# MechaCritter/Python-Visual-Similarity

Hardware: AMD Instinct MI355X
Metric: images/sec encoded + top-k retrieved, VLAD K256 RootSIFT (higher is better)
Workload: dtype f32

## Files before the change

include/pvsim.h:

```cpp
#ifndef PVSIM_H
#define PVSIM_H

#include <stddef.h>
#include <stdint.h>

#ifdef __cplusplus
extern "C" {
#endif

#define PVS_VERSION 103

typedef enum {
  PVS_OK = 0,
  PVS_ERR_INVALID = 1,
  PVS_ERR_NO_DEVICE = 2,
  PVS_ERR_OOM = 3,
  PVS_ERR_UNSUPPORTED = 4,
  PVS_ERR_DIM = 5
} pvs_status;

typedef enum {
  PVS_DESC_F32 = 0,
  PVS_DESC_F32_ROOTSIFT = 1,
  PVS_DESC_U8_ROOTSIFT = 2
} pvs_desc_kind;

typedef enum {
  PVS_OPT_ASSIGN_PREFILTER = 0,
  PVS_OPT_VLAD_PATH = 1,
  PVS_OPT_TOPK_SELECT_ONLY = 2,
  PVS_OPT_AGG_VARIANT = 3,
  PVS_OPT_FISHER_SCALE = 4,
  PVS_OPT_COUNT_ = 5
} pvs_option;

typedef struct pvs_ctx pvs_ctx;
typedef struct pvs_codebook pvs_codebook;
typedef struct pvs_gmm pvs_gmm;
typedef struct pvs_pca pvs_pca;
typedef struct pvs_comm pvs_comm;

typedef struct {
  double power_norm_weight;
  double norm_order;
  double epsilon;
} pvs_norm_params;

int pvs_version(void);
const char* pvs_last_error(void);
int pvs_device_count(int* count);
int pvs_init(int device_id, void* stream, pvs_ctx** out);
int pvs_destroy(pvs_ctx* ctx);
int pvs_sync(pvs_ctx* ctx);
void* pvs_stream(pvs_ctx* ctx);
int pvs_device_name(pvs_ctx* ctx, char* buf, size_t buflen);
int pvs_set_option(pvs_ctx* ctx, int option, int value);
int pvs_get_option(pvs_ctx* ctx, int option, int* value);

int pvs_malloc(pvs_ctx* ctx, size_t bytes, void** dptr);
int pvs_free(pvs_ctx* ctx, void* dptr);
int pvs_memcpy_h2d(pvs_ctx* ctx, void* dst_dev, const void* src_host, size_t bytes);
int pvs_memcpy_d2h(pvs_ctx* ctx, void* dst_host, const void* src_dev, size_t bytes);
int pvs_memset(pvs_ctx* ctx, void* dst_dev, int value, size_t bytes);

int pvs_fill_dev(pvs_ctx* ctx, void* dst_dev, int64_t n_elems, int elem_bytes, uint64_t pattern);
int pvs_stream_wait(pvs_ctx* waiter, pvs_ctx* signal);

int pvs_codebook_create(pvs_ctx* ctx, const float* centroids , int K, int D, pvs_codebook** out);
int pvs_codebook_destroy(pvs_ctx* ctx, pvs_codebook* cb);
int pvs_gmm_create(pvs_ctx* ctx, const double* weights , const double* means ,
                   const double* covariances , int K, int D, pvs_gmm** out);
int pvs_gmm_destroy(pvs_ctx* ctx, pvs_gmm* g);
int pvs_pca_create(pvs_ctx* ctx, const float* components , const float* mean ,
                   int n_components, int d_in, pvs_pca** out);
int pvs_pca_destroy(pvs_ctx* ctx, pvs_pca* p);

int pvs_vlad_encode(pvs_ctx* ctx, const pvs_codebook* cb, const pvs_pca* pca, const void* desc,
                    int desc_kind, const int64_t* offsets, int64_t n_images, const pvs_norm_params* prm,
                    float* out, int32_t* out_labels);
int pvs_vlad_encode_dev(pvs_ctx* ctx, const pvs_codebook* cb, const pvs_pca* pca, const void* d_desc,
                        int desc_kind, const int64_t* d_offsets, int64_t n_images, int64_t total_desc,
                        const pvs_norm_params* prm, float* d_out, int32_t* d_labels, float* d_inv_norm);
int pvs_kmeans_predict_dev(pvs_ctx* ctx, const pvs_codebook* cb, const void* d_desc, int desc_kind,
                           int64_t total_desc, int32_t* d_labels);

int pvs_fisher_encode(pvs_ctx* ctx, const pvs_gmm* g, const pvs_pca* pca, const void* desc, int desc_kind,
                      const int64_t* offsets, int64_t n_images, const pvs_norm_params* prm, double* out);
int pvs_fisher_encode_dev(pvs_ctx* ctx, const pvs_gmm* g, const pvs_pca* pca, const void* d_desc,
                          int desc_kind, const int64_t* d_offsets, int64_t n_images, int64_t total_desc,
                          const pvs_norm_params* prm, void* d_out, int out_f64);
int pvs_gmm_predict_proba_dev(pvs_ctx* ctx, const pvs_gmm* g, const void* d_desc, int desc_kind,
                              int64_t total_desc, double* d_resp);
int pvs_pca_transform_dev(pvs_ctx* ctx, const pvs_pca* p, const void* d_desc, int desc_kind,
                          int64_t total_desc, float* d_out);

int pvs_cosine(pvs_ctx* ctx, const void* A, int64_t M, const void* B, int64_t N, int64_t L, int is_f64,
               void* out );
int pvs_row_inv_norms_dev(pvs_ctx* ctx, const float* d_x, int64_t rows, int64_t L, float* d_inv);
int pvs_cosine_dev(pvs_ctx* ctx, const float* d_A, int64_t M, const float* d_B, int64_t N, int64_t L,
                   const float* d_inv_a, const float* d_inv_b, float* d_out, int64_t ldo);

int pvs_cosine_dual_dev(pvs_ctx* ctx, const float* d_A, int64_t M, const float* d_B, int64_t N, int64_t L,
                        const float* d_inv_a, const float* d_inv_b, float* d_out, int64_t ldo, float* d_out_t, int64_t ldt);

int pvs_topk_dev(pvs_ctx* ctx, const float* d_scores, int64_t nq, int64_t ncols, int64_t ld, int k,
                 int64_t col_offset, int merge, int64_t* d_idx, float* d_val);
int pvs_cosine_topk_dev(pvs_ctx* ctx, const float* d_Q, int64_t nq, const float* d_DB, int64_t N, int64_t L,
                        const float* d_inv_q, const float* d_inv_db, int k, int64_t col_offset, int merge,
                        int64_t* d_idx, float* d_val);
int pvs_f32_to_f16_dev(pvs_ctx* ctx, const float* d_src, int64_t n, void* d_dst_f16);
int pvs_cosine_f16_dev(pvs_ctx* ctx, const void* d_A16, int64_t M, const void* d_B16, int64_t N, int64_t L,
                       const float* d_inv_a, const float* d_inv_b, float* d_out, int64_t ldo);
int pvs_cosine_topk_f16_dev(pvs_ctx* ctx, const void* d_Q16, int64_t nq, const void* d_DB16, int64_t N, int64_t L,
                            const float* d_inv_q, const float* d_inv_db, int k, int64_t col_offset, int merge,
                            int64_t* d_idx, float* d_val);
int pvs_cosine_topk(pvs_ctx* ctx, const float* Q, int64_t nq, const float* DB, int64_t N, int64_t L, int k,
// ... 62 lines not shown
```

python-visual-similarity_amd/csrc/common.hpp:

```cpp
#pragma once
#include <hip/hip_runtime.h>

#include <cmath>
#include <cstdarg>
#include <cstdint>
#include <cstdio>
#include <cstring>
#include <map>
#include <vector>

#include "../../include/pvsim.h"
#include "../../include/pvsim_diag.h"

#define PVS_EXPORT extern "C" __attribute__((visibility("default")))

namespace pvs {

void set_error(const char* fmt, ...);

#define PVS_FAIL(code, ...)        \
  do {                             \
    ::pvs::set_error(__VA_ARGS__); \
    return (code);                 \
  } while (0)

#define PVS_HIP(expr)                                                                    \
  do {                                                                                   \
    hipError_t e__ = (expr);                                                             \
    if (e__ != hipSuccess) {                                                             \
      ::pvs::set_error("%s failed: %s (%s:%d)", #expr, hipGetErrorString(e__), __FILE__, \
                       __LINE__);                                                        \
      return e__ == hipErrorOutOfMemory ? PVS_ERR_OOM : PVS_ERR_NO_DEVICE;               \
    }                                                                                    \
  } while (0)

#define PVS_TRY(expr)                 \
  do {                                \
    int s__ = (expr);                 \
    if (s__ != PVS_OK) return s__;    \
  } while (0)

constexpr int WAVE = 64;

enum TimerSlot { T_ASSIGN = 0, T_AGGREGATE = 1, T_GEMM = 2, T_TOPK = 3, T_FPOST = 4, T_FMOM = 5, T_MISC = 6, T_RESCORE = 7 };

struct TimerRec {
  hipEvent_t a, b;
  int slot;
};

}

struct pvs_ctx {
  int device = 0;
  hipStream_t stream = nullptr;
  bool owns_stream = false;
  int num_cu = 256;
  static constexpr int NWS = 9;
  void* ws[NWS] = {};
  size_t ws_bytes[NWS] = {};
  struct GemmPlanSlot {
    int key[4] = {-1, -1, -1, -1};
    int n_main = 0, n_tail = 0, splitk = 1;
    void* d_tiles = nullptr;
    size_t cap = 0;
  } gemm_plan[5];
  std::map<const void*, int> lds_attr;
  int opt[PVS_OPT_COUNT_] = {1, 0, 0, 0, 0};
  unsigned int* d_queue = nullptr;
  unsigned long long* d_fused_stamps = nullptr;
  bool timers_on = false;
  std::vector<pvs::TimerRec> pending;
  std::vector<hipEvent_t> event_pool;
  std::multimap<size_t, void*> block_cache;
  std::map<void*, size_t> block_size;
  size_t block_cache_bytes = 0;
  void* h_stage = nullptr;
  size_t h_stage_bytes = 0;
  double t_total[PVS_TIMER_SLOTS] = {0};
  int64_t t_count[PVS_TIMER_SLOTS] = {0};
};

struct pvs_codebook {
  int K = 0, D = 0;
  int K_pad = 0, D_pad = 0;
  float* d_cent = nullptr;
  float* d_cpad = nullptr;
  float* d_cnorm = nullptr;
  void* d_c16 = nullptr;
  int D_pad16 = 0;
  int c16_shift = 0;
  float cmax = 0.f;
  void* d_cnk = nullptr;
  void* d_c16n = nullptr;
  int cn_e1 = 0;
};

struct pvs_gmm {
  int K = 0, D = 0;
  double* d_w = nullptr;
  double* d_mu = nullptr;
  double* d_cov = nullptr;
  double* d_prec = nullptr;
  double* d_mup = nullptr;
  double* d_inv_mu = nullptr;
  double* d_inv_sg = nullptr;
  double* d_const = nullptr;
};

struct pvs_pca {
  int C = 0, Din = 0;
  float* d_comp = nullptr;
  float* d_off = nullptr;
};

namespace pvs {

int ws_reserve(pvs_ctx* ctx, int which, size_t bytes, void** out);

inline int ensure_lds(pvs_ctx* ctx, const void* fn, size_t bytes) {
  auto it = ctx->lds_attr.find(fn);
  if (it == ctx->lds_attr.end() || it->second < (int)bytes) {
    PVS_HIP(hipFuncSetAttribute(fn, hipFuncAttributeMaxDynamicSharedMemorySize, (int)bytes));
    ctx->lds_attr[fn] = (int)bytes;
  }
  return PVS_OK;
}

struct ScopedTimer {
  pvs_ctx* ctx;
  int slot;
  hipEvent_t a = nullptr, b = nullptr;
  hipEvent_t take_event() {
    if (!ctx->event_pool.empty()) {
      hipEvent_t e = ctx->event_pool.back();
      ctx->event_pool.pop_back();
      return e;
    }
    hipEvent_t e = nullptr;
    return hipEventCreate(&e) == hipSuccess ? e : nullptr;
  }
  ScopedTimer(pvs_ctx* c, int s) : ctx(c), slot(s) {
    if (ctx->timers_on) {
      if (ctx->pending.size() >= 128) {
        size_t done = 0;
        while (done < ctx->pending.size() && hipEventQuery(ctx->pending[done].b) == hipSuccess) {
          float ms = 0.f;
          if (hipEventElapsedTime(&ms, ctx->pending[done].a, ctx->pending[done].b) == hipSuccess) {
            ctx->t_total[ctx->pending[done].slot] += ms;
            ctx->t_count[ctx->pending[done].slot] += 1;
          }
// ... 78 lines not shown
```

python-visual-similarity_amd/csrc/vlad.hip:

```cpp
#include "common.hpp"
#include "desc_load.hpp"

namespace pvs {

typedef float f32x16 __attribute__((ext_vector_type(16)));

struct AssignArgs {
  const void* X;
  int64_t total;
  int D, ld;
  const float* Cpad;
  const float* cnorm;
  int K_pad, D_pad;
  int32_t* labels;
  const int64_t* rows;
  const unsigned long long* nrows;
  int64_t rows_cap;
};

constexpr int ASSIGN_THREADS = 512;
constexpr int ASSIGN_ROWS = (ASSIGN_THREADS / 64) * 32;
constexpr int ASSIGN_DCHUNK = 128;

template <int NT, int KIND, bool VEC>
__global__ __launch_bounds__(ASSIGN_THREADS, 2) void assign_kernel(AssignArgs a) {
  extern __shared__ __attribute__((aligned(16))) char smem[];
  constexpr int CB = 32 * NT;
  const int cw_max = a.D_pad < ASSIGN_DCHUNK ? a.D_pad : ASSIGN_DCHUNK;
  const int stride = cw_max + 4;
  float* lds_c = reinterpret_cast<float*>(smem);
  float* lds_n = lds_c + CB * stride;

  const int lane = threadIdx.x & 63, wave = threadIdx.x >> 6;
  const int j = lane & 31, h = lane >> 5;
  const int ncb = a.K_pad / CB;
  const int nsc = (a.D_pad + ASSIGN_DCHUNK - 1) / ASSIGN_DCHUNK;
  const bool restage = (ncb * nsc) > 1;
  const int64_t n_items = a.rows ? (int64_t)a.nrows[blockIdx.x] : a.total;
  const int64_t nblocks = (n_items + ASSIGN_ROWS - 1) / ASSIGN_ROWS;
  const int64_t* const my_rows = a.rows ? a.rows + (int64_t)blockIdx.x * a.rows_cap : nullptr;

  auto stage = [&](int cb, int sc) {
    const int cw = min(ASSIGN_DCHUNK, a.D_pad - sc * ASSIGN_DCHUNK);
    const int c4n = cw >> 2;
    for (int idx = threadIdx.x; idx < CB * c4n; idx += ASSIGN_THREADS) {
      const int r = idx / c4n, c4 = idx - r * c4n;
      const float4 v = *reinterpret_cast<const float4*>(a.Cpad + (int64_t)(cb * CB + r) * a.D_pad +
                                                        sc * ASSIGN_DCHUNK + 4 * c4);
      *reinterpret_cast<float4*>(lds_c + r * stride + 4 * c4) = v;
    }
    for (int idx = threadIdx.x; idx < CB; idx += ASSIGN_THREADS) lds_n[idx] = a.cnorm[cb * CB + idx];
  };

  if (!restage) {
    stage(0, 0);
    __syncthreads();
  }

  for (int64_t blk = my_rows ? 0 : blockIdx.x; blk < nblocks; blk += my_rows ? 1 : gridDim.x) {
    const int64_t item = blk * ASSIGN_ROWS + wave * 32 + j;
    const bool rvalid = item < n_items;
    const int64_t row = (my_rows && rvalid) ? my_rows[item] : item;
    float best = INFINITY;
    int bidx = 0;

    for (int cb = 0; cb < ncb; ++cb) {
      f32x16 acc[NT];
#pragma unroll
      for (int t = 0; t < NT; ++t)
#pragma unroll
        for (int r = 0; r < 16; ++r) acc[t][r] = 0.f;

      for (int sc = 0; sc < nsc; ++sc) {
        if (restage) {
          __syncthreads();
          stage(cb, sc);
          __syncthreads();
        }
        const int dc = sc * ASSIGN_DCHUNK;
        const int nt = min(ASSIGN_DCHUNK, a.D_pad - dc) >> 3;

        float4 xb[16];
#pragma unroll
        for (int t = 0; t < 16; ++t) {
          xb[t] = make_float4(0.f, 0.f, 0.f, 0.f);
          if (t < nt) {
            const int d = dc + 8 * t + 4 * h;
            if constexpr (VEC) {
              if (rvalid && d < a.D) xb[t] = load4<KIND>(a.X, row, a.ld, d);
            } else {
              if (rvalid) {
                if (d + 0 < a.D) xb[t].x = load1<KIND>(a.X, row, a.ld, d + 0);
                if (d + 1 < a.D) xb[t].y = load1<KIND>(a.X, row, a.ld, d + 1);
                if (d + 2 < a.D) xb[t].z = load1<KIND>(a.X, row, a.ld, d + 2);
                if (d + 3 < a.D) xb[t].w = load1<KIND>(a.X, row, a.ld, d + 3);
              }
            }
          }
        }
        if constexpr (DescTraits<KIND>::rootsift) {
          float s = 0.f;
#pragma unroll
          for (int t = 0; t < 16; ++t) s += (xb[t].x + xb[t].y) + (xb[t].z + xb[t].w);
          s += __shfl_xor(s, 32, 64);
          const RootsiftRow<KIND> rr(s);
#pragma unroll
          for (int t = 0; t < 16; ++t) {
            xb[t].x = rr(xb[t].x);
            xb[t].y = rr(xb[t].y);
            xb[t].z = rr(xb[t].z);
            xb[t].w = rr(xb[t].w);
          }
        }

#pragma unroll
        for (int t = 0; t < 16; ++t) {
          if (t < nt) {
#pragma unroll
            for (int tile = 0; tile < NT; ++tile) {
              const float4 c4 =
                  *reinterpret_cast<const float4*>(lds_c + (32 * tile + j) * stride + 8 * t + 4 * h);
// ... 655 lines not shown
            for (int tile = 0; tile < 2; ++tile)
#pragma unroll
              for (int f = 0; f < 2; ++f)
                acc[ab][tile][f] = __builtin_amdgcn_mfma_f32_16x16x32_f16(fl[buf][tile], xh[f][s], s == 0 ? zero4 : acc[ab][tile][f], 0, 0, 0);
          }
          if constexpr (NP >= 2) {
#pragma unroll
            for (int tile = 0; tile < 2; ++tile)
#pragma unroll
              for (int f = 0; f < 2; ++f)
                acc[ab][tile][f] = __builtin_amdgcn_mfma_f32_16x16x32_f16(fh[buf][tile], xl[f][s], (NP == 2 && s == 0) ? zero4 : acc[ab][tile][f], 0, 0, 0);
          }
#pragma unroll
          for (int tile = 0; tile < 2; ++tile)
#pragma unroll
            for (int f = 0; f < 2; ++f)
              acc[ab][tile][f] = __builtin_amdgcn_mfma_f32_16x16x32_f16(fh[buf][tile], xh[f][s], (NP == 1 && s == 0) ? zero4 : acc[ab][tile][f], 0, 0, 0);
          if (s == 3) {
#pragma unroll
            for (int tile = 0; tile < 2; ++tile) {
              const f16x4_t pk = *reinterpret_cast<const f16x4_t*>(lds_k + 4 * (32 * gr + 16 * tile + j));
              f16x8_t ca;
#pragma unroll
              for (int q = 0; q < 8; ++q) ca[q] = (_Float16)0.f;
              if constexpr (LUT) {
                if (g == 0) { ca[0] = pk[0]; ca[1] = pk[0]; ca[2] = pk[1]; ca[3] = pk[1]; ca[4] = pk[2]; ca[5] = pk[2]; }
              } else {
                if (g == 0) { ca[0] = pk[0]; ca[1] = pk[1]; ca[2] = pk[2]; }
              }
#pragma unroll
              for (int f = 0; f < 2; ++f)
                acc[ab][tile][f] = __builtin_amdgcn_mfma_f32_16x16x32_f16(ca, cnb[f], acc[ab][tile][f], 0, 0, 0);
            }
          }
          if (gr > 0) select4(ab ^ 1, gr - 1, s);
          __builtin_amdgcn_sched_barrier(0);
        }
      }
    }
#pragma unroll
    for (int part = 0; part < 4; ++part) select4(1, 7, part);
    __builtin_amdgcn_s_barrier();

#pragma unroll
    for (int f = 0; f < 2; ++f) {
      const float m2s = -2.f * ldexpf(1.f, -(x_shift[f] + a.c_shift));
      float b = best[f] * m2s, sc = second[f] * m2s;
      int bi = bidx[f] + 4 * g;
#pragma unroll
      for (int m = 16; m <= 32; m <<= 1) {
        const float ob = __shfl_xor(b, m, 64), os = __shfl_xor(sc, m, 64);
        const int oi = __shfl_xor(bi, m, 64);
        const bool take = ob < b || (ob == b && oi < bi);
        const float nb = take ? ob : b, loser = take ? b : ob;
        sc = fminf(fminf(sc, os), loser);
        b = nb;
        if (take) bi = oi;
      }
      const float xc = nx[f] * a.cmax;
      constexpr float conv_err = DescTraits<KIND>::rootsift ? 4.8e-7f : 0.f;
      const float cc = LUT ? a.cmax * a.cmax * lut_sd[f] : a.cmax * a.cmax;
      constexpr float drop_err = (3 - NP) * 4.9e-4f;
      const float eps = 2.f * (4.8e-7f + 2.4e-7f + 4.8e-5f + 7.7e-6f + 1e-9f + conv_err + drop_err) * xc * (1.f + sqrt_d * 1e-9f) + (LUT ? 6.0e-7f : 2.4e-7f) * (cc + 2.f * xc);
      const bool settled = !(sc <= b + 2.f * eps) && finite[f] && fabsf(b) <= 3.0e38f && bi < a.K;
      const int64_t row = blk * ASSIGN_ROWS + wave * 32 + 16 * f + j;
      const bool amb = g == 0 && rvalid[f] && !settled;
      const unsigned long long amask = __ballot(amb);
      unsigned int base = 0;
      if (amask != 0ull) {
        if (lane == 0) base = atomicAdd(&s_count, (unsigned int)__popcll(amask));
        base = __shfl(base, 0, 64);
      }
      if (g == 0 && rvalid[f]) {
        if (settled) a.labels[row] = bi;
        else my_rows[base + __popcll(amask & ((1ull << lane) - 1ull))] = row;
      }
    }
  }
  if (!pp_g1) __builtin_amdgcn_s_barrier();
  __syncthreads();
  if (threadIdx.x == 0) a.amb_count[blockIdx.x] = s_count;
}

template <int NT, int KIND>
static int launch_assign_nt(pvs_ctx* ctx, const AssignArgs& a, bool vec, size_t lds, int grid) {
  auto kv = assign_kernel<NT, KIND, true>;
  auto ks = assign_kernel<NT, KIND, false>;
  auto k = vec ? kv : ks;
  PVS_HIP(hipFuncSetAttribute(reinterpret_cast<const void*>(k), hipFuncAttributeMaxDynamicSharedMemorySize,
                              (int)lds));
  hipLaunchKernelGGL(k, dim3(grid), dim3(ASSIGN_THREADS), lds, ctx->stream, a);
  PVS_HIP(hipGetLastError());
  return PVS_OK;
}

template <int KIND>
static int launch_assign_kind(pvs_ctx* ctx, const AssignArgs& a, int nt, bool vec, size_t lds, int grid) {
  switch (nt) {
    case 8: return launch_assign_nt<8, KIND>(ctx, a, vec, lds, grid);
    case 4: return launch_assign_nt<4, KIND>(ctx, a, vec, lds, grid);
    case 2: return launch_assign_nt<2, KIND>(ctx, a, vec, lds, grid);
    default: return launch_assign_nt<1, KIND>(ctx, a, vec, lds, grid);
  }
}

template <int NT, int KIND>
static int launch_assign16_nt(pvs_ctx* ctx, const Assign16Args& p, bool vec, size_t lds, int grid) {
  auto kv = assign16_kernel<NT, KIND, true, 0>;
  auto ks = assign16_kernel<NT, KIND, false, 0>;
  auto k8 = assign16_kernel<NT, KIND, true, 8>;
  auto k = vec ? (p.D == 128 && p.D_pad16 == 128 ? k8 : kv) : ks;
  if constexpr (NT == 8) {
    if (k == k8 && p.nprod == 3 && p.shape16 && p.stamps == nullptr) k = assign16x_kernel<KIND, 3>;
  }
  if constexpr (NT == 8) {
    if (k == k8 && p.nprod == 2) k = assign16_kernel<NT, KIND, true, 8, false, 2>;
    if (k == k8 && p.nprod == 1) k = assign16_kernel<NT, KIND, true, 8, false, 1>;
  }
  if constexpr (NT == 8) {
    if (p.stamps != nullptr && k == k8) k = assign16_kernel<NT, KIND, true, 8, true>;
  }
  PVS_HIP(hipFuncSetAttribute(reinterpret_cast<const void*>(k), hipFuncAttributeMaxDynamicSharedMemorySize, (int)lds));
  hipLaunchKernelGGL(k, dim3(grid), dim3(ASSIGN_THREADS), lds, ctx->stream, p);
  PVS_HIP(hipGetLastError());
  return PVS_OK;
}
template <int KIND>
static int launch_assign16_kind(pvs_ctx* ctx, const Assign16Args& p, int nt, bool vec, size_t lds, int grid) {
  switch (nt) {
    case 8: return launch_assign16_nt<8, KIND>(ctx, p, vec, lds, grid);
    case 4: return launch_assign16_nt<4, KIND>(ctx, p, vec, lds, grid);
    case 2: return launch_assign16_nt<2, KIND>(ctx, p, vec, lds, grid);
    case 1: return launch_assign16_nt<1, KIND>(ctx, p, vec, lds, grid);
    default: PVS_FAIL(PVS_ERR_INVALID, "assignment prefilter: unexpected table padding");
  }
}
static int launch_assign16(pvs_ctx* ctx, const Assign16Args& p, int kind, int nt, bool vec, size_t lds, int grid) {
  switch (kind) {
    case PVS_DESC_F32: return launch_assign16_kind<PVS_DESC_F32>(ctx, p, nt, vec, lds, grid);
    case PVS_DESC_F32_ROOTSIFT: return launch_assign16_kind<PVS_DESC_F32_ROOTSIFT>(ctx, p, nt, vec, lds, grid);
    case PVS_DESC_U8_ROOTSIFT: return launch_assign16_kind<PVS_DESC_U8_ROOTSIFT>(ctx, p, nt, vec, lds, grid);
    default: PVS_FAIL(PVS_ERR_INVALID, "unknown descriptor kind %d", kind);
  }
}

int assign_tiles_for(int K) {
  const int k32 = (K + 31) / 32 * 32;
  return k32 > 128 ? 8 : (k32 > 64 ? 4 : (k32 > 32 ? 2 : 1));
}

int launch_assign(pvs_ctx* ctx, const pvs_codebook* cb, const void* d_desc, int kind, int64_t total, int ld,
                  int32_t* d_labels, const float2** rowstat_out) {
  if (rowstat_out) *rowstat_out = nullptr;
  if (total <= 0) return PVS_OK;
  const bool rs = kind != PVS_DESC_F32;
  if (rs && cb->D > ASSIGN_DCHUNK)
    PVS_FAIL(PVS_ERR_UNSUPPORTED, "fused RootSIFT needs D <= %d (got %d)", ASSIGN_DCHUNK, cb->D);
  const int nt = assign_tiles_for(cb->K);
  if (cb->K_pad % (32 * nt) != 0) PVS_FAIL(PVS_ERR_INVALID, "codebook padding does not match the tile count");
  AssignArgs a{d_desc, total, cb->D, ld, cb->d_cpad, cb->d_cnorm, cb->K_pad, cb->D_pad, d_labels, nullptr, nullptr, 0};
  const int esz = kind == PVS_DESC_U8_ROOTSIFT ? 1 : 4;
  const bool vec = (cb->D % 4 == 0) && (ld % 4 == 0) && ((reinterpret_cast<uintptr_t>(d_desc) % (4 * esz)) == 0);
  const int cw = cb->D_pad < ASSIGN_DCHUNK ? cb->D_pad : ASSIGN_DCHUNK;
  const size_t lds = (size_t)(32 * nt) * (cw + 4) * 4 + (size_t)(32 * nt) * 4;
  const int64_t nblocks = (total + ASSIGN_ROWS - 1) / ASSIGN_ROWS;
  const int grid = (int)(nblocks < ctx->num_cu ? nblocks : ctx->num_cu);
  ScopedTimer tm(ctx, T_ASSIGN);
  const bool pre = cb->d_c16 != nullptr && total >= 4096 && ctx->opt[PVS_OPT_ASSIGN_PREFILTER] != 0;
  if (pre) {
    const int64_t cap = (nblocks + grid - 1) / grid * ASSIGN_ROWS;
    char* ws = nullptr;
    const size_t cnt_b = ((size_t)grid * 8 + 255) / 256 * 256;
    const bool stat = rowstat_out != nullptr && kind == PVS_DESC_U8_ROOTSIFT;
    const size_t list_b = ((size_t)grid * cap * 8 + 255) / 256 * 256;
    PVS_TRY(ws_reserve(ctx, 6, cnt_b + list_b + (stat ? (size_t)total * sizeof(float2) : 0), reinterpret_cast<void**>(&ws)));
    unsigned long long* cnt = reinterpret_cast<unsigned long long*>(ws);
    int64_t* rows = reinterpret_cast<int64_t*>(ws + cnt_b);
    float2* rowstat = stat ? reinterpret_cast<float2*>(ws + cnt_b + list_b) : nullptr;
    if (stat) *rowstat_out = rowstat;
    Assign16Args p{d_desc, total, cb->D, ld, static_cast<const _Float16*>(cb->d_c16), cb->d_cnorm, cb->K_pad, cb->D_pad16,
                   cb->c16_shift, cb->cmax, static_cast<const _Float16*>(cb->d_cnk), cb->cn_e1, cb->K, d_labels, rows, cnt, cap, rowstat,
                   ctx->d_fused_stamps, ctx->opt[PVS_OPT_ASSIGN_PREFILTER] == 2 ? 2 : (ctx->opt[PVS_OPT_ASSIGN_PREFILTER] == 3 ? 1 : 3),
                   ctx->opt[PVS_OPT_ASSIGN_PREFILTER] == 4 ? 1 : 0};
    const size_t lds16 = (size_t)2 * cb->K_pad * (128 + 8) * 2 + (size_t)cb->K_pad * 4 + (size_t)cb->K_pad * 8 + 1024;
    PVS_TRY(launch_assign16(ctx, p, kind, cb->K_pad / 32, vec, lds16, grid));
    a.rows = rows;
    a.nrows = cnt;
    a.rows_cap = cap;
  }
  switch (kind) {
    case PVS_DESC_F32: return launch_assign_kind<PVS_DESC_F32>(ctx, a, nt, vec, lds, grid);
    case PVS_DESC_F32_ROOTSIFT: return launch_assign_kind<PVS_DESC_F32_ROOTSIFT>(ctx, a, nt, vec, lds, grid);
    case PVS_DESC_U8_ROOTSIFT: return launch_assign_kind<PVS_DESC_U8_ROOTSIFT>(ctx, a, nt, vec, lds, grid);
    default: PVS_FAIL(PVS_ERR_INVALID, "unknown descriptor kind %d", kind);
  }
}

struct AggArgs {
  const void* X;
  int D, ld;
  const int64_t* offsets;
  const int32_t* labels;
  const float* cent;
  int K;
  float power, eps;
  int norm_mode;
  float norm_p;
  float* out;
  float* inv_norm;
  const float2* rowstat;
};

constexpr int AGG_THREADS = 256;
constexpr int AGG_WAVES = AGG_THREADS / 64;
constexpr int AGG_CHUNK = 4096;

template <int KIND, int GROUP, int VW, int NREG, bool HIOCC = false>
__global__ __launch_bounds__(AGG_THREADS, (HIOCC ? 8 : 1)) void vlad_aggregate_kernel(AggArgs a) {
  extern __shared__ __attribute__((aligned(16))) char smem[];
  const int K = a.K, D = a.D;
  int* hist = reinterpret_cast<int*>(smem);
  int* start = hist + AGG_WAVES * K;
  float* rowsq = reinterpret_cast<float*>(start + K + 1);
  int* scan_tmp = reinterpret_cast<int*>(rowsq + K);
  uint16_t* order = reinterpret_cast<uint16_t*>(scan_tmp + AGG_WAVES);

  const int img = blockIdx.x;
  const int tid = threadIdx.x, lane = tid & 63, wave = tid >> 6;
  const int64_t row0 = a.offsets[img];
  const int64_t n = a.offsets[img + 1] - row0;
  float* out_img = a.out + (int64_t)img * K * D;

  constexpr int NGROUPS = AGG_THREADS / GROUP;
  const int grp = tid / GROUP, gl = tid % GROUP;
  int kbits = 0;
  while ((1 << kbits) < K) ++kbits;

  const int64_t nchunks = n > 0 ? (n + AGG_CHUNK - 1) / AGG_CHUNK : 1;
  for (int64_t ch = 0; ch < nchunks; ++ch) {
    const int64_t cbase = row0 + ch * AGG_CHUNK;
    const int cn = (int)min((int64_t)AGG_CHUNK, n - ch * AGG_CHUNK);
    const bool last = (ch == nchunks - 1);

    for (int i = tid; i < AGG_WAVES * K; i += AGG_THREADS) hist[i] = 0;
    __syncthreads();
    const int per_wave = (cn + AGG_WAVES - 1) / AGG_WAVES;
    const int wbeg = min(cn, wave * per_wave), wend = min(cn, wbeg + per_wave);
    for (int i = wbeg + lane; i < wend; i += 64) atomicAdd(&hist[wave * K + a.labels[cbase + i]], 1);
    __syncthreads();

    {
      int carry = 0;
      for (int k0 = 0; k0 < K; k0 += AGG_THREADS) {
        const int k = k0 + tid;
        int c[AGG_WAVES], tot = 0;
#pragma unroll
        for (int w = 0; w < AGG_WAVES; ++w) {
          c[w] = k < K ? hist[w * K + k] : 0;
          tot += c[w];
        }
        int incl = tot;
#pragma unroll
        for (int d = 1; d < 64; d <<= 1) {
          const int o = __shfl_up(incl, d, 64);
          if (lane >= d) incl += o;
        }
        if (lane == 63) scan_tmp[wave] = incl;
        __syncthreads();
// ... 464 lines not shown
```

python-visual-similarity_amd/pvsim/_ffi.py:

```python
from __future__ import annotations

import ctypes as C
import os
import threading

import numpy as np

_HERE = os.path.dirname(os.path.abspath(__file__))
LIB_PATH = os.environ.get("PVSIM_LIB", os.path.join(_HERE, "libpvsim_hip.so"))

PVS_OK, PVS_ERR_INVALID, PVS_ERR_NO_DEVICE, PVS_ERR_OOM, PVS_ERR_UNSUPPORTED, PVS_ERR_DIM = range(6)
_EXC = {PVS_ERR_INVALID: ValueError, PVS_ERR_NO_DEVICE: RuntimeError, PVS_ERR_OOM: MemoryError,
        PVS_ERR_UNSUPPORTED: NotImplementedError, PVS_ERR_DIM: RuntimeError}

DESC_F32, DESC_F32_ROOTSIFT, DESC_U8_ROOTSIFT = 0, 1, 2
OPT_ASSIGN_PREFILTER, OPT_VLAD_PATH, OPT_TOPK_SELECT_ONLY, OPT_AGG_VARIANT, OPT_FISHER_SCALE = 0, 1, 2, 3, 4
VLAD_PATH_AUTO, VLAD_PATH_GATHER, VLAD_PATH_STREAM, VLAD_PATH_FUSED = 0, 1, 2, 3
TIMER_NAMES = ("assign", "aggregate", "cosine_gemm", "topk", "fisher_posterior", "fisher_moments", "misc", "rescore")


class NormParams(C.Structure):
    _fields_ = [("power_norm_weight", C.c_double), ("norm_order", C.c_double), ("epsilon", C.c_double)]


_vp, _i64, _int, _sz = C.c_void_p, C.c_int64, C.c_int, C.c_size_t
_pp = C.POINTER(C.c_void_p)
_np = C.POINTER(NormParams)

SIGNATURES = {
    "pvs_version": [],
    "pvs_last_error": [],
    "pvs_device_count": [C.POINTER(C.c_int)],
    "pvs_init": [_int, _vp, _pp],
    "pvs_destroy": [_vp],
    "pvs_sync": [_vp],
    "pvs_stream": [_vp],
    "pvs_device_name": [_vp, C.c_char_p, _sz],
    "pvs_set_option": [_vp, _int, _int],
    "pvs_get_option": [_vp, _int, C.POINTER(C.c_int)],
    "pvs_malloc": [_vp, _sz, _pp],
    "pvs_free": [_vp, _vp],
    "pvs_memcpy_h2d": [_vp, _vp, _vp, _sz],
    "pvs_memcpy_d2h": [_vp, _vp, _vp, _sz],
    "pvs_memset": [_vp, _vp, _int, _sz],
    "pvs_fill_dev": [_vp, _vp, _i64, _int, C.c_uint64],
    "pvs_stream_wait": [_vp, _vp],
    "pvs_comm_unique_id": [_vp],
    "pvs_comm_init": [_vp, _int, _int, _vp, _pp],
    "pvs_comm_destroy": [_vp],
    "pvs_comm_library": [],
    "pvs_allgather_dev": [_vp, _vp, _vp, _sz],
    "pvs_alltoall_dev": [_vp, _vp, _vp, _sz],
    "pvs_sendrecv_dev": [_vp, _int, _vp, _vp, _vp, _vp, _vp],
    "pvs_allreduce_max_f64": [_vp, _vp, _int],
    "pvs_comm_barrier": [_vp],
    "pvs_codebook_create": [_vp, _vp, _int, _int, _pp],
    "pvs_codebook_destroy": [_vp, _vp],
    "pvs_gmm_create": [_vp, _vp, _vp, _vp, _int, _int, _pp],
    "pvs_gmm_destroy": [_vp, _vp],
    "pvs_pca_create": [_vp, _vp, _vp, _int, _int, _pp],
    "pvs_pca_destroy": [_vp, _vp],
    "pvs_vlad_encode": [_vp, _vp, _vp, _vp, _int, _vp, _i64, _np, _vp, _vp],
    "pvs_vlad_encode_dev": [_vp, _vp, _vp, _vp, _int, _vp, _i64, _i64, _np, _vp, _vp, _vp],
    "pvs_kmeans_predict_dev": [_vp, _vp, _vp, _int, _i64, _vp],
    "pvs_fisher_encode": [_vp, _vp, _vp, _vp, _int, _vp, _i64, _np, _vp],
    "pvs_fisher_encode_dev": [_vp, _vp, _vp, _vp, _int, _vp, _i64, _i64, _np, _vp, _int],
    "pvs_gmm_predict_proba_dev": [_vp, _vp, _vp, _int, _i64, _vp],
    "pvs_pca_transform_dev": [_vp, _vp, _vp, _int, _i64, _vp],
    "pvs_cosine": [_vp, _vp, _i64, _vp, _i64, _i64, _int, _vp],
    "pvs_row_inv_norms_dev": [_vp, _vp, _i64, _i64, _vp],
    "pvs_cosine_dev": [_vp, _vp, _i64, _vp, _i64, _i64, _vp, _vp, _vp, _i64],
    "pvs_cosine_dual_dev": [_vp, _vp, _i64, _vp, _i64, _i64, _vp, _vp, _vp, _i64, _vp, _i64],
    "pvs_topk_dev": [_vp, _vp, _i64, _i64, _i64, _int, _i64, _int, _vp, _vp],
    "pvs_cosine_topk_dev": [_vp, _vp, _i64, _vp, _i64, _i64, _vp, _vp, _int, _i64, _int, _vp, _vp],
    "pvs_cosine_topk_filtered_dev": [_vp, _vp, _i64, _vp, _i64, _i64, _vp, _vp, _int, _vp, _vp, _vp],
    "pvs_f32_to_f16_dev": [_vp, _vp, _i64, _vp],
    "pvs_cosine_f16_dev": [_vp, _vp, _i64, _vp, _i64, _i64, _vp, _vp, _vp, _i64],
    "pvs_cosine_topk_f16_dev": [_vp, _vp, _i64, _vp, _i64, _i64, _vp, _vp, _int, _i64, _int, _vp, _vp],
    "pvs_cosine_topk": [_vp, _vp, _i64, _vp, _i64, _i64, _int, _vp, _vp],
    "pvs_cosine_topk_f64": [_vp, _vp, _i64, _vp, _i64, _i64, _int, _vp, _vp],
    "pvs_row_inv_norms_f64_dev": [_vp, _vp, _i64, _i64, _vp],
    "pvs_cosine_f64_dev": [_vp, _vp, _i64, _vp, _i64, _i64, _vp, _vp, _vp, _i64],
    "pvs_cosine_topk_f64_dev": [_vp, _vp, _i64, _vp, _i64, _i64, _vp, _vp, _int, _vp, _vp],
    "pvs_topk_merge_dev": [_vp, _vp, _vp, _int, _i64, _int, _vp, _vp],
    "pvs_materialise_dev": [_vp, _vp, _int, _int, _i64, _vp],
    "pvs_kmeans_step_dev": [_vp, _vp, _vp, _i64, _vp, _vp, _vp, _vp],
    "pvs_gmm_em_step_dev": [_vp, _vp, _vp, _i64, _vp],
    "pvs_label_sums_dev": [_vp, _vp, _int, _i64, _vp, _int, _int, _vp],
    "pvs_gram_dev": [_vp, _vp, _int, _i64, _vp],
    "pvs_seed_distances_dev": [_vp, _vp, _int, _i64, _vp, _int, _vp, _vp, _vp, _int],
    "pvs_seed_pick_dev": [_vp, _vp, _int, _i64, _vp, _vp, _vp, _vp, _int, _vp, _vp],
    "pvs_min_update_dev": [_vp, _vp, _vp, _i64, _vp],
    "pvs_kmeanspp_run_dev": [_vp, _vp, _int, _i64, _int, _int, _vp, _vp],
    "pvs_l2_knn_dev": [_vp, _vp, _i64, _vp, _i64, _i64, _int, _int, _vp, _vp, _vp],
    "pvs_l2_radius_count_dev": [_vp, _vp, _i64, _vp, _i64, _i64, _int, C.c_double, _vp],
    "pvs_l2_radius_fill_dev": [_vp, _vp, _i64, _vp, _i64, _i64, _int, C.c_double, _vp, _vp, _vp],
    "pvs_csr_spmm_f64_dev": [_vp, _i64, _vp, _vp, _vp, _vp, _int, C.c_double, _vp, _vp, C.c_double, _vp],
    "pvs_transpose_f64_dev": [_vp, _vp, _i64, _i64, _vp],
    "pvs_fused_profile": [_vp, _int, _vp],
# ... 79 lines not shown
```

Before: 420,600.

## Add near-tie refinement pass to resolve ambiguous assignment rows cheaply

```diff
diff --git a/include/pvsim.h b/include/pvsim.h
--- a/include/pvsim.h
+++ b/include/pvsim.h
@@ -31,7 +31,8 @@
   PVS_OPT_TOPK_SELECT_ONLY = 2,
   PVS_OPT_AGG_VARIANT = 3,
   PVS_OPT_FISHER_SCALE = 4,
-  PVS_OPT_COUNT_ = 5
+  PVS_OPT_ASSIGN_NEAR = 5,
+  PVS_OPT_COUNT_ = 6
 } pvs_option;
 
 typedef struct pvs_ctx pvs_ctx;
diff --git a/python-visual-similarity_amd/csrc/common.hpp b/python-visual-similarity_amd/csrc/common.hpp
--- a/python-visual-similarity_amd/csrc/common.hpp
+++ b/python-visual-similarity_amd/csrc/common.hpp
@@ -66,7 +66,7 @@
     size_t cap = 0;
   } gemm_plan[5];
   std::map<const void*, int> lds_attr;
-  int opt[PVS_OPT_COUNT_] = {1, 0, 0, 0, 0};
+  int opt[PVS_OPT_COUNT_] = {1, 0, 0, 0, 0, 1};
   unsigned int* d_queue = nullptr;
   unsigned long long* d_fused_stamps = nullptr;
   bool timers_on = false;
diff --git a/python-visual-similarity_amd/csrc/vlad.hip b/python-visual-similarity_amd/csrc/vlad.hip
--- a/python-visual-similarity_amd/csrc/vlad.hip
+++ b/python-visual-similarity_amd/csrc/vlad.hip
@@ -37,6 +37,7 @@
   const int nsc = (a.D_pad + ASSIGN_DCHUNK - 1) / ASSIGN_DCHUNK;
   const bool restage = (ncb * nsc) > 1;
   const int64_t n_items = a.rows ? (int64_t)a.nrows[blockIdx.x] : a.total;
+  if (n_items == 0) return;
   const int64_t nblocks = (n_items + ASSIGN_ROWS - 1) / ASSIGN_ROWS;
   const int64_t* const my_rows = a.rows ? a.rows + (int64_t)blockIdx.x * a.rows_cap : nullptr;
 
@@ -858,6 +859,249 @@
   if (threadIdx.x == 0) a.amb_count[blockIdx.x] = s_count;
 }
 
+constexpr int NEAR_CAP = 16;
+
+struct NearArgs {
+  const void* X;
+  int D, ld;
+  const _Float16* C16;
+  const float* Cpad;
+  const float* cnorm;
+  int K_pad, K;
+  int c_shift;
+  float cmax;
+  int32_t* labels;
+  int64_t* rows;
+  unsigned long long* nrows;
+  int64_t rows_cap;
+};
+
+template <int NT, int KIND>
+__global__ __launch_bounds__(ASSIGN_THREADS, 1) void assign_near_kernel(NearArgs a) {
+  extern __shared__ __attribute__((aligned(16))) char smem[];
+  __shared__ unsigned int s_left;
+  __shared__ int s_pairs[(ASSIGN_THREADS / 64) * 32 * NEAR_CAP];
+  constexpr int CB = 32 * NT;
+  constexpr int stride = 128 + 8;
+  _Float16* lds_h = reinterpret_cast<_Float16*>(smem);
+  _Float16* lds_l = lds_h + CB * stride;
+  float* lds_n = reinterpret_cast<float*>(lds_l + CB * stride);
+  const int lane = threadIdx.x & 63, wave = threadIdx.x >> 6;
+  const int j = lane & 31, h = lane >> 5;
+  const int64_t n_items = (int64_t)a.nrows[blockIdx.x];
+  if (n_items == 0) return;
+  int64_t* const my_rows = a.rows + (int64_t)blockIdx.x * a.rows_cap;
+
+  for (int idx = threadIdx.x; idx < 2 * CB * 16; idx += ASSIGN_THREADS) {
+    const int r = idx >> 4, c8 = idx & 15;
+    *reinterpret_cast<uint4*>(lds_h + r * stride + 8 * c8) = *reinterpret_cast<const uint4*>(a.C16 + (int64_t)r * 128 + 8 * c8);
+  }
+  for (int idx = threadIdx.x; idx < CB; idx += ASSIGN_THREADS) lds_n[idx] = a.cnorm[idx];
+  if (threadIdx.x == 0) s_left = 0u;
+
+  const float sqrt_d = sqrtf(128.f);
+  const int64_t nblocks = (n_items + ASSIGN_ROWS - 1) / ASSIGN_ROWS;
+  for (int64_t blk = 0; blk < nblocks; ++blk) {
+    const int64_t item = blk * ASSIGN_ROWS + wave * 32 + j;
+    const bool rvalid = item < n_items;
+    const int64_t row = rvalid ? my_rows[item] : 0;
+    __syncthreads();
+
+    float xf[8][8];
+#pragma unroll
+    for (int t = 0; t < 8; ++t) {
+#pragma unroll
+      for (int q = 0; q < 8; ++q) xf[t][q] = 0.f;
+      if (rvalid) {
+        const float4 v0 = load4<KIND>(a.X, row, a.ld, 16 * t + 4 * h);
+        const float4 v1 = load4<KIND>(a.X, row, a.ld, 16 * t + 4 * h + 8);
+        xf[t][0] = v0.x; xf[t][1] = v0.y; xf[t][2] = v0.z; xf[t][3] = v0.w;
+        xf[t][4] = v1.x; xf[t][5] = v1.y; xf[t][6] = v1.z; xf[t][7] = v1.w;
+      }
+    }
+    float rsum = 0.f;
+    if constexpr (DescTraits<KIND>::rootsift) {
+#pragma unroll
+      for (int t = 0; t < 8; ++t) {
+        rsum += (xf[t][0] + xf[t][1]) + (xf[t][2] + xf[t][3]);
+        rsum += (xf[t][4] + xf[t][5]) + (xf[t][6] + xf[t][7]);
+      }
+      rsum += __shfl_xor(rsum, 32, 64);
+      const RootsiftRow<KIND> rr(rsum);
+#pragma unroll
+      for (int t = 0; t < 8; ++t) {
+#pragma unroll
+        for (int q = 0; q < 8; ++q) xf[t][q] = rr(xf[t][q]);
+        __builtin_amdgcn_sched_barrier(0);
+      }
+    }
+
+    float n2 = 0.f, amax = 0.f;
+#pragma unroll
+    for (int t = 0; t < 8; ++t)
+#pragma unroll
+      for (int q = 0; q < 8; ++q) {
+        n2 = fmaf(xf[t][q], xf[t][q], n2);
+        amax = fmaxf(amax, fabsf(xf[t][q]));
+      }
+    n2 += __shfl_xor(n2, 32, 64);
+    amax = fmaxf(amax, __shfl_xor(amax, 32, 64));
+    const float nx = sqrtf(n2) * 1.0001f;
+    int ex = 13;
+    if (amax > 0.f) (void)frexpf(amax, &ex);
+    int x_shift = 13 - ex;
+    bool finite = nx <= 3.0e38f;
+    if (x_shift > 40 || x_shift < -40) { finite = false; x_shift = 0; }
+    const float xs = ldexpf(1.f, x_shift);
+    f16x8_t xh[8], xl[8];
+#pragma unroll
+    for (int t = 0; t < 8; ++t)
+#pragma unroll
+      for (int q = 0; q < 8; ++q) {
+        const float v = xf[t][q] * xs;
+        const _Float16 hi = (_Float16)v;
+        xh[t][q] = hi;
+        xl[t][q] = (_Float16)(v - (float)hi);
+      }
+    f32x16 acc[NT];
+#pragma unroll
+    for (int tile = 0; tile < NT; ++tile)
+#pragma unroll
+      for (int r = 0; r < 16; ++r) acc[tile][r] = 0.f;
+#pragma unroll
+    for (int t = 0; t < 8; ++t)
+#pragma unroll
+      for (int tile = 0; tile < NT; ++tile) {
+        const f16x8_t ch = *reinterpret_cast<const f16x8_t*>(lds_h + (32 * tile + j) * stride + 16 * t + 8 * h);
+        const f16x8_t cl = *reinterpret_cast<const f16x8_t*>(lds_l + (32 * tile + j) * stride + 16 * t + 8 * h);
+        acc[tile] = __builtin_amdgcn_mfma_f32_32x32x16_f16(cl, xh[t], acc[tile], 0, 0, 0);
+        acc[tile] = __builtin_amdgcn_mfma_f32_32x32x16_f16(ch, xl[t], acc[tile], 0, 0, 0);
+        acc[tile] = __builtin_amdgcn_mfma_f32_32x32x16_f16(ch, xh[t], acc[tile], 0, 0, 0);
+        __builtin_amdgcn_sched_barrier(0);
+      }
+    const float m2s = -2.f * ldexpf(1.f, -(x_shift + a.c_shift));
+    float best = INFINITY;
+#pragma unroll
+    for (int tile = 0; tile < NT; ++tile) {
+#pragma unroll
+      for (int g = 0; g < 4; ++g) {
+        const float4 cn = *reinterpret_cast<const float4*>(lds_n + 32 * tile + 8 * g + 4 * h);
+        acc[tile][4 * g + 0] = fmaf(m2s, acc[tile][4 * g + 0], cn.x);
+        acc[tile][4 * g + 1] = fmaf(m2s, acc[tile][4 * g + 1], cn.y);
+        acc[tile][4 * g + 2] = fmaf(m2s, acc[tile][4 * g + 2], cn.z);
+        acc[tile][4 * g + 3] = fmaf(m2s, acc[tile][4 * g + 3], cn.w);
+        best = fminf(best, fminf(fminf(acc[tile][4 * g + 0], acc[tile][4 * g + 1]), fminf(acc[tile][4 * g + 2], acc[tile][4 * g + 3])));
+      }
+      __builtin_amdgcn_sched_barrier(0);
+    }
+    best = fminf(best, __shfl_xor(best, 32, 64));
+
+    const float xc = nx * a.cmax;
+    const float eps = 2.f * (4.8e-7f + 2.4e-7f + 4.8e-5f + 7.7e-6f + 1e-9f) * xc * (1.f + sqrt_d * 1e-9f) + 2.4e-7f * (a.cmax * a.cmax + 2.f * xc);
+    const float thr = best + 2.5f * eps;
+    uint32_t cmask[(NT + 1) / 2];
+#pragma unroll
+    for (int w = 0; w < (NT + 1) / 2; ++w) cmask[w] = 0u;
+#pragma unroll
+    for (int tile = 0; tile < NT; ++tile)
+#pragma unroll
+      for (int r = 0; r < 16; ++r)
+        if (acc[tile][r] <= thr) cmask[tile >> 1] |= 1u << (16 * (tile & 1) + r);
+    int ncand = 0;
+#pragma unroll
+    for (int w = 0; w < (NT + 1) / 2; ++w) ncand += __popc(cmask[w]);
+    ncand += __shfl_xor(ncand, 32, 64);
+    const bool open = rvalid && finite && fabsf(best) <= 3.0e38f && ncand <= NEAR_CAP;
+    if (!open) {
+#pragma unroll
+      for (int w = 0; w < (NT + 1) / 2; ++w) cmask[w] = 0u;
+    }
+
+    int nown = 0;
+#pragma unroll
+    for (int w = 0; w < (NT + 1) / 2; ++w) nown += __popc(cmask[w]);
+    int incl = nown;
+#pragma unroll
+    for (int d = 1; d < 64; d <<= 1) {
+      const int o = __shfl_up(incl, d, 64);
+      if (lane >= d) incl += o;
+    }
+    const int pbase = incl - nown;
+    const int npairs = __shfl(incl, 63, 64);
+    int* const s_pair = s_pairs + wave * (32 * NEAR_CAP);
+    {
+      int e = pbase;
+#pragma unroll
+      for (int w = 0; w < (NT + 1) / 2; ++w) {
+        uint32_t m = cmask[w];
+        while (m != 0u) {
+          const int p = __builtin_ctz(m);
+          m &= m - 1u;
+          const int r = p & 15, k = 32 * (2 * w + (p >> 4)) + 8 * (r >> 2) + 4 * h + (r & 3);
+          s_pair[e++] = j | (k << 8);
+        }
+      }
+    }
+    __syncthreads();
+    __builtin_amdgcn_sched_barrier(0);
+    for (int e0 = 0; e0 < npairs; e0 += 64) {
+      const int e = e0 + lane;
+      const int ent = e < npairs ? s_pair[e] : 0;
+      const int pj = ent & 31, k = ent >> 8;
+      const int64_t prow = __shfl(row, pj, 64);
+      const float psum = __shfl(rsum, pj, 64);
+      if (e < npairs) {
+        const RootsiftRow<KIND> rr(psum);
+        const float* cr = a.Cpad + (int64_t)k * 128;
+        float dot = 0.f;
+#pragma unroll
+        for (int b8 = 0; b8 < 128; b8 += 8) {
+          float4 xa = load4<KIND>(a.X, prow, a.ld, b8), xb = load4<KIND>(a.X, prow, a.ld, b8 + 4);
+          if constexpr (DescTraits<KIND>::rootsift) {
+            xa.x = rr(xa.x); xa.y = rr(xa.y); xa.z = rr(xa.z); xa.w = rr(xa.w);
+            xb.x = rr(xb.x); xb.y = rr(xb.y); xb.z = rr(xb.z); xb.w = rr(xb.w);
+          }
+          const float4 ca = *reinterpret_cast<const float4*>(cr + b8), cb = *reinterpret_cast<const float4*>(cr + b8 + 4);
+          dot = fmaf(ca.x, xa.x, dot); dot = fmaf(cb.x, xb.x, dot);
+          dot = fmaf(ca.y, xa.y, dot); dot = fmaf(cb.y, xb.y, dot);
+          dot = fmaf(ca.z, xa.z, dot); dot = fmaf(cb.z, xb.z, dot);
+          dot = fmaf(ca.w, xa.w, dot); dot = fmaf(cb.w, xb.w, dot);
+          if (DescTraits<KIND>::rootsift || (b8 & 63) == 56) __builtin_amdgcn_sched_barrier(0);
+        }
+        s_pair[e] = __float_as_int(fmaf(-2.f, dot, lds_n[k]));
+      }
+    }
+    __syncthreads();
+    float bv = INFINITY;
+    int bk = 0x7fffffff;
+    {
+      int e = pbase;
+#pragma unroll
+      for (int w = 0; w < (NT + 1) / 2; ++w) {
+        uint32_t m = cmask[w];
+        while (m != 0u) {
+          const int p = __builtin_ctz(m);
+          m &= m - 1u;
+          const int r = p & 15, k = 32 * (2 * w + (p >> 4)) + 8 * (r >> 2) + 4 * h + (r & 3);
+          const float v = __int_as_float(s_pair[e++]);
+          if (v < bv || (v == bv && k < bk)) { bv = v; bk = k; }
+        }
+      }
+    }
+    {
+      const float ov = __shfl_xor(bv, 32, 64);
+      const int ok = __shfl_xor(bk, 32, 64);
+      if (ov < bv || (ov == bv && ok < bk)) { bv = ov; bk = ok; }
+    }
+    if (h == 0 && rvalid) {
+      if (open && bv < INFINITY && bk < a.K) a.labels[row] = bk;
+      else my_rows[atomicAdd(&s_left, 1u)] = row;
+    }
+  }
+  __syncthreads();
+  if (threadIdx.x == 0) a.nrows[blockIdx.x] = s_left;
+}
+
 template <int NT, int KIND>
 static int launch_assign_nt(pvs_ctx* ctx, const AssignArgs& a, bool vec, size_t lds, int grid) {
   auto kv = assign_kernel<NT, KIND, true>;
@@ -909,6 +1153,33 @@
     case 2: return launch_assign16_nt<2, KIND>(ctx, p, vec, lds, grid);
     case 1: return launch_assign16_nt<1, KIND>(ctx, p, vec, lds, grid);
     default: PVS_FAIL(PVS_ERR_INVALID, "assignment prefilter: unexpected table padding");
+  }
+}
+template <int NT, int KIND>
+static int launch_near_nt(pvs_ctx* ctx, const NearArgs& p, int grid) {
+  auto k = assign_near_kernel<NT, KIND>;
+  const size_t lds = (size_t)2 * (32 * NT) * (128 + 8) * 2 + (size_t)(32 * NT) * 4;
+  PVS_HIP(hipFuncSetAttribute(reinterpret_cast<const void*>(k), hipFuncAttributeMaxDynamicSharedMemorySize, (int)lds));
+  hipLaunchKernelGGL(k, dim3(grid), dim3(ASSIGN_THREADS), lds, ctx->stream, p);
+  PVS_HIP(hipGetLastError());
+  return PVS_OK;
+}
+template <int KIND>
+static int launch_near_kind(pvs_ctx* ctx, const NearArgs& p, int nt, int grid) {
+  switch (nt) {
+    case 8: return launch_near_nt<8, KIND>(ctx, p, grid);
+    case 4: return launch_near_nt<4, KIND>(ctx, p, grid);
+    case 2: return launch_near_nt<2, KIND>(ctx, p, grid);
+    case 1: return launch_near_nt<1, KIND>(ctx, p, grid);
+    default: PVS_FAIL(PVS_ERR_INVALID, "near-tie pass: unexpected table padding");
+  }
+}
+static int launch_near(pvs_ctx* ctx, const NearArgs& p, int kind, int nt, int grid) {
+  switch (kind) {
+    case PVS_DESC_F32: return launch_near_kind<PVS_DESC_F32>(ctx, p, nt, grid);
+    case PVS_DESC_F32_ROOTSIFT: return launch_near_kind<PVS_DESC_F32_ROOTSIFT>(ctx, p, nt, grid);
+    case PVS_DESC_U8_ROOTSIFT: return launch_near_kind<PVS_DESC_U8_ROOTSIFT>(ctx, p, nt, grid);
+    default: PVS_FAIL(PVS_ERR_INVALID, "unknown descriptor kind %d", kind);
   }
 }
 static int launch_assign16(pvs_ctx* ctx, const Assign16Args& p, int kind, int nt, bool vec, size_t lds, int grid) {
@@ -960,6 +1231,11 @@
                    ctx->opt[PVS_OPT_ASSIGN_PREFILTER] == 4 ? 1 : 0};
     const size_t lds16 = (size_t)2 * cb->K_pad * (128 + 8) * 2 + (size_t)cb->K_pad * 4 + (size_t)cb->K_pad * 8 + 1024;
     PVS_TRY(launch_assign16(ctx, p, kind, cb->K_pad / 32, vec, lds16, grid));
+    if (ctx->opt[PVS_OPT_ASSIGN_NEAR] != 0 && vec && cb->D == 128 && cb->D_pad == 128 && cb->D_pad16 == 128) {
+      NearArgs q{d_desc, cb->D, ld, static_cast<const _Float16*>(cb->d_c16), cb->d_cpad, cb->d_cnorm, cb->K_pad, cb->K,
+                 cb->c16_shift, cb->cmax, d_labels, rows, cnt, cap};
+      PVS_TRY(launch_near(ctx, q, kind, cb->K_pad / 32, grid));
+    }
     a.rows = rows;
     a.nrows = cnt;
     a.rows_cap = cap;
diff --git a/python-visual-similarity_amd/pvsim/_ffi.py b/python-visual-similarity_amd/pvsim/_ffi.py
--- a/python-visual-similarity_amd/pvsim/_ffi.py
+++ b/python-visual-similarity_amd/pvsim/_ffi.py
@@ -14,7 +14,7 @@
         PVS_ERR_UNSUPPORTED: NotImplementedError, PVS_ERR_DIM: RuntimeError}
 
 DESC_F32, DESC_F32_ROOTSIFT, DESC_U8_ROOTSIFT = 0, 1, 2
-OPT_ASSIGN_PREFILTER, OPT_VLAD_PATH, OPT_TOPK_SELECT_ONLY, OPT_AGG_VARIANT, OPT_FISHER_SCALE = 0, 1, 2, 3, 4
+OPT_ASSIGN_PREFILTER, OPT_VLAD_PATH, OPT_TOPK_SELECT_ONLY, OPT_AGG_VARIANT, OPT_FISHER_SCALE, OPT_ASSIGN_NEAR = 0, 1, 2, 3, 4, 5
 VLAD_PATH_AUTO, VLAD_PATH_GATHER, VLAD_PATH_STREAM, VLAD_PATH_FUSED = 0, 1, 2, 3
 TIMER_NAMES = ("assign", "aggregate", "cosine_gemm", "topk", "fisher_posterior", "fisher_moments", "misc", "rescore")
 
```

New measurement: 421,400 (median of 6 runs). No clear change (+0.2%).
